# NeRdTheNed/deft4j

Hardware: NVIDIA B200
Metric: input MB/s optimised (-m NONE) (higher is better)
Workload: dtype u8

## Files before the change

__graft_entry__.py:

```python
import os
import subprocess
import sys

ROOT = os.path.dirname(os.path.abspath(__file__))
CSRC = os.path.join(ROOT, "deft4j_b200", "csrc")
NVCC = os.environ.get("NVCC", "/usr/local/cuda/bin/nvcc")


def _newer(target, sources):
    if not os.path.exists(target):
        return True
    t = os.path.getmtime(target)
    return any(os.path.exists(s) and os.path.getmtime(s) > t for s in sources)


def build():
    srcs = [os.path.join(CSRC, f) for f in os.listdir(CSRC) if f.endswith((".cu", ".cuh", ".cpp", ".h"))]
    srcs.append(os.path.join(ROOT, "include", "deft4cu.h"))
    lib = os.path.join(ROOT, "deft4j_b200", "libdeft4cu.so")
    if _newer(lib, srcs):
        subprocess.check_call([NVCC, "-gencode", "arch=compute_100a,code=sm_100a", "-O3", "-lineinfo", "-std=c++17",
                               "--shared", "-Xcompiler", "-fPIC,-pthread", "-o", lib, os.path.join(CSRC, "deft4cu.cu"),
                               os.path.join(CSRC, "png_front.cpp"), os.path.join(CSRC, "zip_front.cpp"),
                               os.path.join(CSRC, "gz_front.cpp")])
    small = os.path.join(ROOT, "deft4j_b200", "libdeft4cu_smallpools.so")
    if _newer(small, srcs):
        subprocess.check_call([NVCC, "-gencode", "arch=compute_100a,code=sm_100a", "-O3", "-lineinfo", "-std=c++17",
                               "-DD4_SMALL_POOLS", "--shared", "-Xcompiler", "-fPIC,-pthread", "-o", small,
                               os.path.join(CSRC, "deft4cu.cu"), os.path.join(CSRC, "png_front.cpp"),
                               os.path.join(CSRC, "zip_front.cpp"), os.path.join(CSRC, "gz_front.cpp")])
    stress = os.path.join(ROOT, "deft4j_b200", "libdeft4cu_stress.so")
    if _newer(stress, srcs):
        subprocess.check_call([NVCC, "-gencode", "arch=compute_100a,code=sm_100a", "-O3", "-lineinfo", "-std=c++17",
                               "-DD4_HQS=40", "-DD4_HQL=8", "-DD4_LCN=2", "-DD4_DCN=2", "-DD4_MAXLIT=3",
                               "-DD4_FORCE_BIG_WEIGHTS", "--shared", "-Xcompiler", "-fPIC,-pthread", "-o", stress,
                               os.path.join(CSRC, "deft4cu.cu"), os.path.join(CSRC, "png_front.cpp"),
                               os.path.join(CSRC, "zip_front.cpp"), os.path.join(CSRC, "gz_front.cpp")])
    host = os.path.join(ROOT, "deft4j_b200", "libdeft4cu_hosttest.so")
    if _newer(host, srcs):
        subprocess.check_call([NVCC, "-O2", "-std=c++17", "--shared", "-Xcompiler", "-fPIC", "-Wno-deprecated-gpu-targets",
                               "-o", host, os.path.join(CSRC, "hosttest.cu")])
    subprocess.check_call(["make", "-C", os.path.join(ROOT, "oracle")], stdout=subprocess.DEVNULL)
    sys.path.insert(0, ROOT)
    sys.path.insert(0, os.path.join(ROOT, "tests"))
    import hosttest_lib
    hosttest_lib.front_oracle_lib()
    import deft4j_b200
    from deft4j_b200 import _native
    _native.load()


def smoke():
    sys.path.insert(0, ROOT)
    sys.path.insert(0, os.path.join(ROOT, "tests"))
    import zlib
    import workloads
    import oracle_lib
    from deft4j_b200 import optimise_batch, _native
    if not os.path.exists(_native.LIB_PATH):
        build()
    co = zlib.compressobj(6, zlib.DEFLATED, -15, 8)
    cf = zlib.compressobj(6, zlib.DEFLATED, -15, 8, zlib.Z_FIXED)
    text = workloads.c2_text(60000)
    streams = [co.compress(text) + co.flush(), cf.compress(text[:3000]) + cf.flush()]
    res = optimise_batch(streams, True)
    for raw, r in zip(streams, res):
        assert r["status"] == 0, r
        o = oracle_lib.OracleDeflateStream()
# ... 25 lines not shown
```

deft4j_b200/csrc/deft4cu.cu:

```cuda
#include <algorithm>
#include <cstdio>
#include <cstdlib>
#include <cstring>
#include <memory>
#include <chrono>
#include <mutex>
#include <string>
#include <thread>
#include <vector>

#include "../../include/deft4cu.h"

namespace d4 {
static thread_local std::string g_err;
static void set_error(const std::string& s) { g_err = s; }
}

#include "write.cuh"
#include "checksum.cuh"

namespace d4 {

static int g_device = -1;
static int g_sms = 148;
static bool g_sync_debug = getenv("D4_SYNC") != nullptr;
static uint64_t g_opt_launches = 0;
static std::mutex g_mu;

struct HostTimer {
    const char* what; std::chrono::steady_clock::time_point t0; bool on;
    explicit HostTimer(const char* w) : what(w), t0(std::chrono::steady_clock::now()) { static bool e = getenv("D4_HOST_TIMING") != nullptr; on = e; }
    ~HostTimer() {
        if (on && g_device >= 0) {
            cudaMemPool_t pool;
            uint64_t res = 0, used = 0;
            if (cudaDeviceGetDefaultMemPool(&pool, g_device) == cudaSuccess) {
                cudaMemPoolGetAttribute(pool, cudaMemPoolAttrReservedMemCurrent, &res);
                cudaMemPoolGetAttribute(pool, cudaMemPoolAttrUsedMemCurrent, &used);
            }
            fprintf(stderr, "[deft4cu] pool reserved %7.1f MiB used %7.1f MiB  ", res / 1048576.0, used / 1048576.0);
        }
        if (on) fprintf(stderr, "[deft4cu] %-14s %8.3f ms\n", what, std::chrono::duration<double, std::milli>(std::chrono::steady_clock::now() - t0).count());
// ... 489 lines not shown
        cudaEventElapsedTime(&t, ev[0], ev[1]); ms[0] = t;
        cudaEventElapsedTime(&t, ev[1], ev[2]); ms[1] = t;
        cudaEventElapsedTime(&t, ev[2], ev[3]); ms[2] = t;
        ms[7] = (float)parse_rewalks;
        for (auto& e : ev) cudaEventDestroy(e);
        parsed = true;
        return DEFT4CU_OK;
    }

    unsigned char* scratch_raw = nullptr;
    cudaError_t alloc_scratch(EngScratch& sc, unsigned& grid, uint32_t maxwords, uint64_t maxu) {
        const size_t stride = eng_scratch_layout(sc, maxwords, maxu);
        const size_t align = (size_t)2 << 20;
        size_t freeb = 0, totalb = 0;
        if (cudaMemGetInfo(&freeb, &totalb) == cudaSuccess) {
            cudaMemPool_t pool;
            uint64_t res = 0, used = 0;
            if (cudaDeviceGetDefaultMemPool(&pool, g_device) == cudaSuccess &&
                cudaMemPoolGetAttribute(pool, cudaMemPoolAttrReservedMemCurrent, &res) == cudaSuccess &&
                cudaMemPoolGetAttribute(pool, cudaMemPoolAttrUsedMemCurrent, &used) == cudaSuccess && res > used)
                freeb += (size_t)(res - used);
            const size_t margin = ((size_t)1 << 30) + totalb / 16;
            const size_t fit = freeb > margin + align ? (freeb - margin - align) / stride : 0;
            grid = (unsigned)std::max<size_t>(1, std::min<size_t>(grid, fit));
        }
        cudaError_t e = dalloc(&scratch_raw, stride * grid + align, cs);
        if (e != cudaSuccess) return e;
        sc.slab = (unsigned char*)(((uintptr_t)scratch_raw + align - 1) & ~(uintptr_t)(align - 1));
        if (getenv("D4_POISON")) cudaMemsetAsync(sc.slab, 0x7F, stride * grid, cs);
        return cudaSuccess;
    }
    void free_scratch(EngScratch&) { dfree(scratch_raw, cs); }

    int optimise(uint32_t flags, const std::vector<uint8_t>& selected) {
        HostTimer ht("optimise");
        cudaEvent_t ev[3];
        for (auto& e : ev) cudaEventCreate(&e);
        const int merge = (flags & DEFT4CU_MERGE_BLOCKS) ? 1 : 0;
        if (optimised && nblk_total) {
            BlkSummary* d_summ = nullptr;
            D4_CUDA_CHECK(dalloc(&d_summ, nblk_total, cs));
            LAUNCH(k_state_summary, (unsigned)((nblk_total + 255) / 256), 256, cs, d_bs, d_summ, nblk_total);
            D4_CUDA_CHECK(cudaMemcpyAsync(summ.data(), d_summ, sizeof(BlkSummary) * nblk_total, cudaMemcpyDeviceToHost, cs));
            D4_CUDA_CHECK(cudaStreamSynchronize(cs));
            dfree(d_summ, cs);
        }
        optimised = true;
        std::vector<uint32_t> jobs;
        uint32_t maxsym = 1, maxstream = 1;
        uint64_t maxout = 1, maxstream_out = 1;
        for (uint32_t i = 0; i < n; i++) {
            StreamState& s = sstate[i];
            s.selected = selected[i] && s.status == ST_OK;
            s.saved_bits = 0;
            if (!s.selected) continue;
            uint64_t ssum = 0;
            uint32_t n_alive = 0;
            for (uint32_t k = 0; k < s.n_blocks; k++) n_alive += summ[s.blk_base + k].alive;
            s.cut = s.n_blocks;
            for (uint32_t k = 0; k < s.n_blocks; k++) {
                const BlkSummary& b = summ[s.blk_base + k];
                if (b.alive && b.out_len == 0 && n_alive != 1) { s.cut = k; break; }
            }
            for (uint32_t k = 0; k < s.n_blocks; k++) {
                const BlkSummary& b = summ[s.blk_base + k];
                ssum += b.n_sym;
// ... 2 lines not shown
                    maxsym = std::max(maxsym, b.n_sym);
                    maxout = std::max<uint64_t>(maxout, b.out_len);
                }
            }
            maxstream = (uint32_t)std::max<uint64_t>(maxstream, ssum);
            maxstream_out = std::max<uint64_t>(maxstream_out, infos[i].out_len);
        }
        const bool tracing = g_trace_dev != nullptr;
        if (!tracing) std::stable_sort(jobs.begin(), jobs.end(), [&](uint32_t a, uint32_t b) { return summ[a].n_sym > summ[b].n_sym; });
        D4_CUDA_CHECK(cudaMemcpyAsync(d_sstate, sstate.data(), sizeof(StreamState) * n, cudaMemcpyHostToDevice, cs));
        cudaEventRecord(ev[0], cs);
        if (!jobs.empty()) {
            uint32_t* d_jobs = nullptr;
            unsigned* d_counter = nullptr;
            D4_CUDA_CHECK(dalloc(&d_jobs, jobs.size(), cs));
            D4_CUDA_CHECK(dalloc(&d_counter, 1, cs));
            D4_CUDA_CHECK(cudaMemsetAsync(d_counter, 0, 4, cs));
            D4_CUDA_CHECK(cudaMemcpyAsync(d_jobs, jobs.data(), 4 * jobs.size(), cudaMemcpyHostToDevice, cs));
            int perSM = 0;
            cudaFuncSetAttribute(k_opt_blocks, cudaFuncAttributePreferredSharedMemoryCarveout, cudaSharedmemCarveoutMaxShared);
            D4_CUDA_CHECK(cudaOccupancyMaxActiveBlocksPerMultiprocessor(&perSM, k_opt_blocks, ENG_NT, 0));
            if (perSM < 1) perSM = 1;
            if (const char* e = getenv("D4_CTAS_PER_SM")) perSM = std::max(1, std::min(perSM, atoi(e)));
            unsigned grid = (unsigned)std::min<uint64_t>(jobs.size(), (uint64_t)g_sms * perSM);
            if (tracing) grid = 1;
            EngScratch sc{};
            D4_CUDA_CHECK(alloc_scratch(sc, grid, (maxsym + 31) / 32 + 1, maxout));
            g_opt_launches++;
            LAUNCH(k_opt_blocks, grid, ENG_NT, cs, d_jobs, (uint32_t)jobs.size(), d_bs, d_logs, d_sym, d_symout, d_out, d_maskpool, sc, d_counter, d_gerr);
            free_scratch(sc);
            dfree(d_jobs, cs); dfree(d_counter, cs);
        }
        cudaEventRecord(ev[1], cs);
        {
            EngScratch sc{};
            int perSM = 0;
            cudaFuncSetAttribute(k_finish, cudaFuncAttributePreferredSharedMemoryCarveout, cudaSharedmemCarveoutMaxShared);
            D4_CUDA_CHECK(cudaOccupancyMaxActiveBlocksPerMultiprocessor(&perSM, k_finish, ENG_NT, 0));
            if (perSM < 1) perSM = 1;
            unsigned grid = (unsigned)std::min<uint64_t>(n, (uint64_t)g_sms * perSM);
            unsigned* d_counter = nullptr;
            D4_CUDA_CHECK(dalloc(&d_counter, 1, cs));
            D4_CUDA_CHECK(cudaMemsetAsync(d_counter, 0, 4, cs));
            if (merge) D4_CUDA_CHECK(alloc_scratch(sc, grid, (maxstream + 31) / 32 + 2, maxstream_out));
            if (n) LAUNCH(k_finish, grid, ENG_NT, cs, d_sstate, n, d_bs, d_logs, d_sym, d_symout, d_out, d_maskpool, sc, merge, d_counter, d_gerr);
            if (merge) free_scratch(sc);
            dfree(d_counter, cs);
        }
        cudaEventRecord(ev[2], cs);
        int gerrv[8] = {0};
        D4_CUDA_CHECK(cudaMemcpyAsync(sstate.data(), d_sstate, sizeof(StreamState) * n, cudaMemcpyDeviceToHost, cs));
        D4_CUDA_CHECK(cudaMemcpyAsync(gerrv, d_gerr, sizeof(gerrv), cudaMemcpyDeviceToHost, cs));
        D4_CUDA_CHECK(cudaStreamSynchronize(cs));
        float t;
        cudaEventElapsedTime(&t, ev[0], ev[1]); ms[3] = t;
        cudaEventElapsedTime(&t, ev[1], ev[2]); ms[4] = t;
        for (auto& e : ev) cudaEventDestroy(e);
        const int gerr = gerrv[0];
        if (gerr == 13 || gerr == 14) {
            char msg[256];
            snprintf(msg, sizeof msg, "engine self-check: block %d round %d winner idx %d selected size %d, materialised size %d (check %d: 1 "
                     "incumbent != previous winner, 2 payload, 3 size; previous %d; %zu jobs)",
                     gerrv[1], gerrv[2], gerrv[3], gerrv[4], gerrv[5], gerrv[6], gerrv[7], jobs.size());
            set_error(msg);
            return DEFT4CU_ERR_CUDA;
        }
        if (gerr) {
            set_error(gerr == ERR_ROUNDS ? "optimiser hit an internal limit: more than 64 optimiseBlock rounds on one block"
                      : gerr == ERR_POOL ? "optimiser: internal table pool overflow"
                      : gerr == ERR_INTERNAL ? "optimiser: enumerator/executor protocol error (internal)"
                                         : "optimiser: a Huffman tree could not be balanced (the reference throws here)");
            D4_CUDA_CHECK(cudaMemsetAsync(d_gerr, 0, sizeof(int), cs));
            for (uint32_t i = 0; i < n; i++) if (sstate[i].selected) sstate[i].status = ST_UNSUPPORTED;
            return DEFT4CU_ERR_UNSUPPORTED;
        }
        dfree(d_dst, cs);
        h_dst.clear();
        return DEFT4CU_OK;
    }

// ... 503 lines not shown
```

deft4j_b200/csrc/optimise.cuh:

```cuda
#pragma once
#include "engine.cuh"

namespace d4 {

constexpr int MAXR = 64;

struct BlkState {
    Cand cand;
    uint64_t sym_off;
    uint64_t out_off;
    uint64_t mask_off;
    uint64_t out_len;
    uint32_t n_sym;
    int32_t alive;
    int32_t bfinal;
    int32_t nrounds;
    uint64_t bit_pos;
    long long size_bits;
};
struct RoundRec { long long sizeI, sizeC1, restMin, best; };
struct RoundLog { RoundRec r[MAXR]; };

struct StreamState {
    uint64_t blk_base;
// ... 86 lines not shown
                e.pass_hist_full(SLOT_BEST);
                const long long truePay = e.hist_payload(S.hist, e.recs[1].tab);
                if (truePay != e.recs[1].payload) { bad = true; badWhat = 2; }
                if (cand_size(e.recs[1]) != S.en.bestSize) { bad = true; badWhat = 3; }
            }
            if (bad && tid == 0) {
                if (atomicMax(gerr, 13) < 13) {
                    gerr[1] = (int)jobs[job]; gerr[2] = r; gerr[3] = (int)S.en.bestIndex;
                    gerr[4] = (int)S.en.bestSize; gerr[5] = (int)cand_size(e.recs[1]); gerr[6] = badWhat; gerr[7] = (int)prevBest;
                }
            }
            __syncthreads();
            prevBest = S.en.bestSize;
            r++;
            if (!improved) break;
            if (r >= MAXR) { if (tid == 0) S.err = ERR_ROUNDS; break; }
            e.advance_to_best();
        }
        __syncthreads();
        if (r > 1 && !S.err) {
            const uint32_t* s = (const uint32_t*)&e.recs[0];
            uint32_t* d = (uint32_t*)&b.cand;
            for (int k = tid; k < (int)(sizeof(Cand) / 4); k += ENG_NT) d[k] = s[k];
            e.store_mask(SLOT_B, maskpool + b.mask_off);
        }
        if (tid == 0) b.nrounds = r;
        __syncthreads();
        if (S.err) { if (tid == 0) { atomicMax(gerr, S.err); S.err = 0; } }
        __syncthreads();
        P1(PR_BLOCK);
    }
}

__device__ void finish_stream(EngSmem& S, Eng& e, StreamState& st, BlkState* __restrict__ bs, const RoundLog* __restrict__ logs,
                              uint32_t* __restrict__ sym, const uint32_t* __restrict__ symout, const uint8_t* __restrict__ out,
                              uint32_t* __restrict__ maskpool, int merge, int* __restrict__ gerr) {
    __shared__ long long s_pos, s_saved;
    __shared__ int s_cur, s_next, s_do, s_first;
    if (!st.selected || st.status != ST_OK) return;
    const int tid = threadIdx.x;
    BlkState* B = bs + st.blk_base;
    const uint32_t nb = st.n_blocks;

    {
        constexpr int RT = 64, RR = 4;
        struct Tile { unsigned long long out_len[RT]; int type[RT]; RoundRec rr[RT][RR]; };
        static_assert(sizeof(Tile) <= sizeof(EngSmem), "replay tile must fit in the engine's shared storage");
        Tile& T = *reinterpret_cast<Tile*>(&S);
        __shared__ long long s_rpos, s_rsaved;
        __shared__ int s_stop;
        __shared__ uint32_t s_first_alive, s_n_alive;
        if (tid == 0) { s_rpos = 0; s_rsaved = 0; s_stop = 0; s_first_alive = nb; s_n_alive = 0; }
        __syncthreads();
        {
            uint32_t fa = nb, na = 0;
            for (uint32_t k = tid; k < nb; k += ENG_NT) if (B[k].alive) { if (fa == nb) fa = k; na++; }
            if (na) { atomicMin(&s_first_alive, fa); atomicAdd(&s_n_alive, na); }
        }
        __syncthreads();
        const uint32_t first_alive = s_first_alive, n_alive = s_n_alive;
        for (uint32_t t0 = 0; t0 < nb && !s_stop; t0 += RT) {
            const uint32_t cnt = nb - t0 < RT ? nb - t0 : RT;
            for (uint32_t k = tid; k < cnt; k += ENG_NT) {
                T.out_len[k] = B[t0 + k].out_len;
                T.type[k] = B[t0 + k].alive ? (int)B[t0 + k].cand.tab.type : -1;
            }
            for (uint32_t q = tid; q < cnt * RR; q += ENG_NT) T.rr[q / RR][q % RR] = logs[st.blk_base + t0 + q / RR].r[q % RR];
            __syncthreads();
            if (tid == 0) {
                long long pos = s_rpos, saved = s_rsaved;
                for (uint32_t kk = 0; kk < cnt; kk++) {
                    const uint32_t k = t0 + kk;
                    const unsigned long long out_len = T.out_len[kk];
                    if (T.type[kk] < 0) continue;
                    if (out_len > 0 || (k == first_alive && n_alive == 1)) {
                        if (T.type[kk] == 0) {
                            pos += 3;
                            pos += stored_size(out_len, pos);
                        } else {
                            const RoundLog& lg = logs[st.blk_base + k];
                            int r = 0;
                            while (true) {
                                pos += 3;
                                const RoundRec rr = r < RR ? T.rr[kk][r] : lg.r[r];
                                const long long I = rr.sizeI, C1 = rr.sizeC1, R = rr.restMin, W = rr.best;
                                const long long m1 = I < C1 ? I : C1;
                                bool storedWins = false;
                                long long Ssz = 0;
                                if (out_len <= 65535) {
                                    Ssz = stored_size(out_len, pos);
                                    storedWins = Ssz < m1 && Ssz <= R;
                                }
                                if (storedWins) {
                                    saved += I - Ssz;
                                    B[k].cand.tab.type = 0;
                                    pos += stored_size(out_len, pos);
                                    pos += 3;
                                    pos += stored_size(out_len, pos);
                                    break;
                                }
                                if (W < I) { saved += I - W; pos += W; r++; continue; }
                                pos += I;
                                break;
                            }
                        }
                    } else {
                        saved += blk_size(B[k], pos + 3) + 3;
                        B[k].alive = 0;
                        if (B[k].cand.tab.type != 0 && B[k].n_sym) sym[B[k].sym_off + B[k].n_sym - 1] = SYM_NOP;
                        s_stop = 1;
                        break;
                    }
                }
                s_rpos = pos; s_rsaved = saved;
            }
            __syncthreads();
        }
        if (tid == 0) { s_saved = s_rsaved; S.err = 0; }
    }
    __syncthreads();

    if (merge) {
        if (tid == 0) {
            s_pos = 0; s_first = 1;
            int c = 0;
            while (c < (int)nb && !B[c].alive) c++;
            s_cur = c;
        }
        __syncthreads();
        while (true) {
            const int cur = s_cur;
            if (cur >= (int)nb) break;
            if (tid == 0) {
                int n = cur + 1;
                while (n < (int)nb && !B[n].alive) n++;
                s_next = n < (int)nb ? n : -1;
                s_do = 0;
                BlkState& c = B[cur];
                if (s_first && s_next < 0) {
                    s_pos += blk_size(c, s_pos + 3) + 3;
                    s_do = 3;
                } else if (c.out_len > 0) {
                    s_pos += 3;
                    if (s_next >= 0) {
                        BlkState& nx = B[s_next];
                        if (c.cand.tab.type == 0) {
                            if (c.out_len + nx.out_len <= 65535) {
                                long long curSize = blk_size(c, s_pos);
                                long long nextSize = blk_size(nx, s_pos + curSize + 3);
                                long long mergedSize = stored_size(c.out_len + nx.out_len, s_pos);
                                long long cs = curSize + 3 + nextSize - mergedSize;
                                if (cs > 0) {
                                    s_saved += cs;
                                    c.out_len += nx.out_len;
                                    c.n_sym = 0;
// ... 46 lines not shown
                }
                __syncthreads();
                if (s_do == 5) {
                    if (!S.en.bestStored) {
                        const uint32_t* s = (const uint32_t*)&e.recs[1];
                        uint32_t* d = (uint32_t*)&c.cand;
                        for (int k = tid; k < (int)(sizeof(Cand) / 4); k += ENG_NT) d[k] = s[k];
                        e.store_mask(SLOT_BEST, maskpool + c.mask_off);
                    }
                    __syncthreads();
                    if (tid == 0) {
                        if (S.en.bestStored) c.cand.tab.type = 0;
                        c.n_sym = span;
                        c.out_len += nx.out_len;
                        nx.alive = 0;
                    }
                } else {
                    if (tid == 0) sym[c.sym_off + nA - 1] = 256;
                }
                __syncthreads();
                if (tid == 0) s_pos += blk_size(c, s_pos);
                action = (s_do == 5) ? 2 : 3;
                __syncthreads();
            }
            if (action == 4) break;
            if (tid == 0) {
                if (action == 3) {
                    s_cur = s_next < 0 ? (int)nb : s_next;
                    s_first = 0;
                }
            }
            __syncthreads();
        }
        if (S.err && tid == 0) { atomicMax(gerr, S.err); S.err = 0; }
    }
    __syncthreads();

    {
        constexpr int LT = 128;
        struct LTile { unsigned long long out_len[LT], bit_pos[LT]; long long csize[LT], size_bits[LT]; int type[LT], alive[LT]; };
        static_assert(sizeof(LTile) <= sizeof(EngSmem), "layout tile must fit in the engine's shared storage");
        __syncthreads();
        LTile& T = *reinterpret_cast<LTile*>(&S);
        __shared__ long long s_size;
        __shared__ int s_last;
        if (tid == 0) { s_size = 0; s_last = -1; }
        __syncthreads();
        for (uint32_t t0 = 0; t0 < nb; t0 += LT) {
            const uint32_t cnt = nb - t0 < LT ? nb - t0 : LT;
            for (uint32_t k = tid; k < cnt; k += ENG_NT) {
                const BlkState& b = B[t0 + k];
                T.out_len[k] = b.out_len; T.type[k] = b.cand.tab.type; T.alive[k] = b.alive; T.csize[k] = cand_size(b.cand);
            }
            __syncthreads();
            if (tid == 0) {
                long long size = s_size;
                int last = s_last;
                for (uint32_t k = 0; k < cnt; k++) {
                    if (!T.alive[k]) continue;
                    T.bit_pos[k] = (unsigned long long)size;
                    size += 3;
                    T.size_bits[k] = T.type[k] == 0 ? stored_size(T.out_len[k], size) : T.csize[k];
                    size += T.size_bits[k];
                    last = (int)(t0 + k);
                }
                s_size = size; s_last = last;
            }
            __syncthreads();
            for (uint32_t k = tid; k < cnt; k += ENG_NT) {
                if (!T.alive[k]) continue;
                BlkState& b = B[t0 + k];
                b.bit_pos = T.bit_pos[k]; b.size_bits = T.size_bits[k]; b.bfinal = 0;
            }
            __syncthreads();
        }
        if (tid == 0) {
            if (s_last >= 0) B[s_last].bfinal = 1;
            st.total_bits = (uint64_t)s_size;
            st.saved_bits = s_saved;
        }
        __syncthreads();
    }
}

__global__ void __launch_bounds__(ENG_NT, D4_ENG_MINB)
k_finish(StreamState* __restrict__ streams, uint32_t nstreams, BlkState* __restrict__ bs, const RoundLog* __restrict__ logs,
         uint32_t* __restrict__ sym, const uint32_t* __restrict__ symout, const uint8_t* __restrict__ out,
         uint32_t* __restrict__ maskpool, EngScratch sc, int merge, unsigned* __restrict__ counter, int* __restrict__ gerr) {
    EngSmem& S = g_es;
    __shared__ uint32_t s_job;
    Eng e;
    if (merge) eng_init(e, sc, blockIdx.x);
    while (true) {
        __syncthreads();
        if (threadIdx.x == 0) s_job = atomicAdd(counter, 1u);
        __syncthreads();
        const uint32_t job = s_job;
        if (job >= nstreams) break;
        finish_stream(S, e, streams[job], bs, logs, sym, symout, out, maskpool, merge, gerr);
    }
}

}
```

deft4j_b200/csrc/write.cuh:

```cuda
#pragma once
#include "optimise.cuh"

namespace d4 {

constexpr int WR_NT = 256;

__device__ __forceinline__ void put_bits(unsigned long long* outw, uint64_t bitpos, unsigned long long bits, int n) {
    if (n == 0) return;
    const uint64_t w = bitpos >> 6;
    const int sh = (int)(bitpos & 63);
    atomicOr(&outw[w], bits << sh);
    if (sh + n > 64) atomicOr(&outw[w + 1], bits >> (64 - sh));
}

__device__ __forceinline__ uint32_t rev_bits(uint32_t code, int len) { return len ? (__brev(code) >> (32 - len)) : 0; }

__device__ inline void build_codes(const uint8_t* lens, int n, uint16_t* codes) {
    int count[16];
    for (int l = 0; l < 16; l++) count[l] = 0;
    for (int i = 0; i < n; i++) count[lens[i] & 15]++;
    uint32_t next[16];
    uint32_t nc = 0;
    int lastShift = 0;
    for (int l = 1; l < 16; l++) {
        next[l] = 0;
        if (count[l] == 0) continue;
        nc <<= (l - lastShift);
        lastShift = l;
        next[l] = nc;
        nc += count[l];
    }
    for (int i = 0; i < n; i++) {
        int l = lens[i];
        codes[i] = l ? (uint16_t)rev_bits(next[l]++, l) : 0;
    }
}

struct WriteSmem {
    uint16_t codeL[MAX_LL], codeD[MAX_D], codeCL[MAX_CL];
    uint8_t L[MAX_LL], D[MAX_D];
    uint32_t warpsum[WR_NT / 32];
    uint64_t base;
};

__global__ void __launch_bounds__(WR_NT)
k_write(const StreamState* __restrict__ streams, const uint32_t* __restrict__ blk_stream, const BlkState* __restrict__ bs,
        const uint32_t* __restrict__ sym, const uint32_t* __restrict__ symout, const uint8_t* __restrict__ out,
        const uint32_t* __restrict__ maskpool, const uint64_t* __restrict__ dst_off, unsigned long long* __restrict__ dstw,
        int* __restrict__ gerr) {
    const BlkState& b = bs[blockIdx.x];
    const uint32_t sid = blk_stream[blockIdx.x];
    if (!b.alive || streams[sid].status != ST_OK) return;
    const int tid = threadIdx.x;
    unsigned long long* dw = dstw + (dst_off[sid] >> 3);
    const uint64_t pos0 = b.bit_pos;
    const int type = b.cand.tab.type;

    if (type == 0) {
        const uint64_t dataByte = ((pos0 + 3 + 7) >> 3) + 4;
        const uint8_t* src = out + b.out_off;
        if (tid == 0) {
            put_bits(dw, pos0, (unsigned long long)(b.bfinal ? 1 : 0), 3);
            uint32_t len = (uint32_t)b.out_len & 0xffff;
            uint32_t hdr = len | ((~len & 0xffff) << 16);
            put_bits(dw, (dataByte - 4) * 8, hdr, 32);
        }
        const uint64_t n = b.out_len;
        for (uint64_t k = (uint64_t)tid * 8; k < n; k += (uint64_t)WR_NT * 8) {
            unsigned long long v = 0;
            int cnt = (int)((n - k) < 8 ? (n - k) : 8);
            for (int j = 0; j < cnt; j++) v |= (unsigned long long)src[k + j] << (8 * j);
            put_bits(dw, (dataByte + k) * 8, v, cnt * 8);
        }
        return;
    }

    __shared__ WriteSmem W;
    for (int k = tid; k < MAX_LL; k += WR_NT) W.L[k] = b.cand.tab.L[k];
    if (tid < MAX_D) W.D[tid] = b.cand.tab.D[tid];
    __syncthreads();
    if (tid == 0) {
        if (type == 1) { W.L[286] = 8; W.L[287] = 8; }
        build_codes(W.L, type == 1 ? 288 : b.cand.tab.nL, W.codeL);
    }
    if (tid == 32) build_codes(W.D, b.cand.tab.nD, W.codeD);
    if (tid == 64 && type == 2) build_codes(b.cand.hdr.CL, 19, W.codeCL);
    __syncthreads();

    if (tid == 0) {
        uint64_t p = pos0;
        put_bits(dw, p, (unsigned long long)((type << 1) | (b.bfinal ? 1 : 0)), 3);
        p += 3;
        if (type == 2) {
            const Hdr& h = b.cand.hdr;
            put_bits(dw, p, (unsigned long long)((b.cand.tab.nL - 257) & 31), 5); p += 5;
            put_bits(dw, p, (unsigned long long)((b.cand.tab.nD - 1) & 31), 5); p += 5;
            put_bits(dw, p, (unsigned long long)((h.ncl - 4) & 15), 4); p += 4;
            for (int i = 0; i < h.ncl; i++) { put_bits(dw, p, h.CL[c_codelen_order[i]], 3); p += 3; }
            for (int i = 0; i < h.np; i++) {
                uint16_t pr = h.pairs[i];
                int s = pair_sym(pr), run = pair_run(pr);
                put_bits(dw, p, W.codeCL[s], h.CL[s]); p += h.CL[s];
                if (run > 0) {
                    int off = s == 18 ? 11 : 3, sz = pair_extra_bits(s);
                    put_bits(dw, p, (unsigned long long)(run - off), sz); p += sz;
                }
            }
            if ((long long)(p - pos0 - 3) != (long long)h.bits) {
                if (atomicMax(gerr, 2) == 0) { gerr[1] = (int)blockIdx.x; gerr[2] = (int)(p - pos0 - 3); gerr[3] = h.bits; gerr[4] = 1; }
            }
        }
        W.base = p;
    }
    __syncthreads();

    const uint32_t* S = sym + b.sym_off;
    const uint32_t* SO = symout + b.sym_off;
    const uint32_t* M = maskpool + b.mask_off;
    const int lane = tid & 31, wid = tid >> 5;
    for (uint32_t base = 0; base < b.n_sym; base += WR_NT) {
        const uint32_t i = base + tid;
        uint32_t s = 0;
        int nbits = 0;
        bool replaced = false;
        if (i < b.n_sym) {
            s = S[i];
            if (!sym_is_match(s)) {
                nbits = (s <= 256) ? W.L[s] : 0;
            } else {
                replaced = (M[i >> 5] >> (i & 31)) & 1;
                if (!replaced) {
                    int ls = sym_lensym(s), ds = dist_sym(sym_dist(s));
                    nbits = W.L[ls] + len_ebits_of(ls) + W.D[ds] + dist_ebits_of(ds);
                } else {
                    const uint8_t* p = out + SO[i];
                    int len = sym_len(s);
                    for (int k = 0; k < len; k++) nbits += W.L[p[k]];
                }
            }
        }
        uint32_t incl = (uint32_t)nbits;
#pragma unroll
        for (int d = 1; d < 32; d <<= 1) {
            uint32_t a = __shfl_up_sync(0xffffffffu, incl, d);
            if (lane >= d) incl += a;
        }
        if (lane == 31) W.warpsum[wid] = incl;
        __syncthreads();
        uint32_t wbase = 0, total = 0;
        for (int k = 0; k < WR_NT / 32; k++) { uint32_t x = W.warpsum[k]; if (k < wid) wbase += x; total += x; }
        uint64_t p = W.base + wbase + incl - (uint32_t)nbits;
        if (i < b.n_sym && nbits) {
            if (!sym_is_match(s)) {
                put_bits(dw, p, W.codeL[s], nbits);
            } else if (!replaced) {
                int ls = sym_lensym(s), dist = sym_dist(s), ds = dist_sym(dist), len = sym_len(s);
                unsigned long long bits = W.codeL[ls];
                int nb = W.L[ls];
                bits |= (unsigned long long)(len - c_len_base[ls - 257]) << nb;
                nb += len_ebits_of(ls);
                bits |= (unsigned long long)W.codeD[ds] << nb;
                nb += W.D[ds];
                bits |= (unsigned long long)(dist - c_dist_base[ds]) << nb;
                nb += dist_ebits_of(ds);
                put_bits(dw, p, bits, nb);
            } else {
                const uint8_t* q = out + SO[i];
                int len = sym_len(s);
                unsigned long long acc = 0;
                int na = 0;
                for (int k = 0; k < len; k++) {
                    int v = q[k], l = W.L[v];
                    if (na + l > 64) { put_bits(dw, p, acc, na); p += na; acc = 0; na = 0; }
                    acc |= (unsigned long long)W.codeL[v] << na;
                    na += l;
                }
                put_bits(dw, p, acc, na);
            }
        }
        __syncthreads();
        if (tid == 0) W.base += total;
        __syncthreads();
    }
    if (tid == 0) {
        if ((long long)(W.base - pos0 - 3) != b.size_bits) {
            if (atomicMax(gerr, 2) == 0) { gerr[1] = (int)blockIdx.x; gerr[2] = (int)(W.base - pos0 - 3); gerr[3] = (int)b.size_bits; gerr[4] = 2; }
        }
    }
}

}
```

Measured before the change: 1338.

## Parallelise replay and layout via residue-map scans; stage bit writes in shared memory

The serial per-stream replay and layout that ran on one thread inside k_finish is replaced by per-block kernels. These compute bit-position-mod-8 transition maps, compose them with a CUB inclusive scan, and use an exclusive sum for block bit offsets. Separately, k_write now stages output bits in a shared-memory buffer using 32-bit shared atomics and flushes whole words with plain stores, falling back to global atomics when a chunk does not fit. The aim is to remove serial single-thread work and heavy global atomicOr traffic, at the cost of several extra launches, temporary allocations and more shared memory per write block.

```diff
diff --git a/__graft_entry__.py b/__graft_entry__.py
--- a/__graft_entry__.py
+++ b/__graft_entry__.py
@@ -33,7 +33,7 @@
     if _newer(stress, srcs):
         subprocess.check_call([NVCC, "-gencode", "arch=compute_100a,code=sm_100a", "-O3", "-lineinfo", "-std=c++17",
                                "-DD4_HQS=40", "-DD4_HQL=8", "-DD4_LCN=2", "-DD4_DCN=2", "-DD4_MAXLIT=3",
-                               "-DD4_FORCE_BIG_WEIGHTS", "--shared", "-Xcompiler", "-fPIC,-pthread", "-o", stress,
+                               "-DD4_FORCE_BIG_WEIGHTS", "-DD4_WR_BUF=8", "--shared", "-Xcompiler", "-fPIC,-pthread", "-o", stress,
                                os.path.join(CSRC, "deft4cu.cu"), os.path.join(CSRC, "png_front.cpp"),
                                os.path.join(CSRC, "zip_front.cpp"), os.path.join(CSRC, "gz_front.cpp")])
     host = os.path.join(ROOT, "deft4j_b200", "libdeft4cu_hosttest.so")
diff --git a/deft4j_b200/csrc/deft4cu.cu b/deft4j_b200/csrc/deft4cu.cu
--- a/deft4j_b200/csrc/deft4cu.cu
+++ b/deft4j_b200/csrc/deft4cu.cu
@@ -8,6 +8,8 @@
 #include <string>
 #include <thread>
 #include <vector>
+
+#include <cub/device/device_scan.cuh>
 
 #include "../../include/deft4cu.h"
 
@@ -563,6 +565,53 @@
     }
     void free_scratch(EngScratch&) { dfree(scratch_raw, cs); }
 
+    int scan_residues(uint32_t* d_map, uint32_t* d_scan) {
+        size_t tb = 0;
+        D4_CUDA_CHECK(cub::DeviceScan::InclusiveScan(nullptr, tb, d_map, d_scan, RmapThen{}, nblk_total, cs));
+        unsigned char* d_tmp = nullptr;
+        D4_CUDA_CHECK(dalloc(&d_tmp, tb, cs));
+        D4_CUDA_CHECK(cub::DeviceScan::InclusiveScan(d_tmp, tb, d_map, d_scan, RmapThen{}, nblk_total, cs));
+        launches++;
+        dfree(d_tmp, cs);
+        return DEFT4CU_OK;
+    }
+    int replay() {
+        const unsigned g = (unsigned)((nblk_total + 255) / 256);
+        ReplayRec* d_rec = nullptr;
+        uint32_t *d_map = nullptr, *d_scan = nullptr;
+        D4_CUDA_CHECK(dalloc(&d_rec, nblk_total, cs));
+        D4_CUDA_CHECK(dalloc(&d_map, nblk_total, cs));
+        D4_CUDA_CHECK(dalloc(&d_scan, nblk_total, cs));
+        LAUNCH(k_replay_map, g, 256, cs, d_sstate, d_blk_stream, d_bs, d_logs, d_rec, d_map, nblk_total);
+        if (int rc = scan_residues(d_map, d_scan)) return rc;
+        LAUNCH(k_replay_apply, g, 256, cs, d_sstate, d_blk_stream, d_bs, d_rec, d_scan, d_sym, nblk_total);
+        dfree(d_rec, cs); dfree(d_map, cs); dfree(d_scan, cs);
+        return DEFT4CU_OK;
+    }
+    int layout() {
+        const unsigned g = (unsigned)((nblk_total + 256) / 256);
+        uint32_t *d_map = nullptr, *d_scan = nullptr;
+        unsigned long long *d_len = nullptr, *d_pos = nullptr;
+        D4_CUDA_CHECK(dalloc(&d_map, nblk_total, cs));
+        D4_CUDA_CHECK(dalloc(&d_scan, nblk_total, cs));
+        D4_CUDA_CHECK(dalloc(&d_len, nblk_total + 1, cs));
+        D4_CUDA_CHECK(dalloc(&d_pos, nblk_total + 1, cs));
+        LAUNCH(k_layout_map, g, 256, cs, d_sstate, d_blk_stream, d_bs, d_map, nblk_total);
+        if (int rc = scan_residues(d_map, d_scan)) return rc;
+        LAUNCH(k_layout_size, g, 256, cs, d_sstate, d_blk_stream, d_bs, d_scan, d_len, nblk_total);
+        size_t tb = 0;
+        D4_CUDA_CHECK(cub::DeviceScan::ExclusiveSum(nullptr, tb, d_len, d_pos, nblk_total + 1, cs));
+        unsigned char* d_tmp = nullptr;
+        D4_CUDA_CHECK(dalloc(&d_tmp, tb, cs));
+        D4_CUDA_CHECK(cub::DeviceScan::ExclusiveSum(d_tmp, tb, d_len, d_pos, nblk_total + 1, cs));
+        launches++;
+        dfree(d_tmp, cs);
+        LAUNCH(k_layout_apply, g, 256, cs, d_sstate, d_blk_stream, d_bs, d_pos, nblk_total);
+        LAUNCH(k_layout_streams, (n + 255) / 256, 256, cs, d_sstate, d_pos, n);
+        dfree(d_map, cs); dfree(d_scan, cs); dfree(d_len, cs); dfree(d_pos, cs);
+        return DEFT4CU_OK;
+    }
+
     int optimise(uint32_t flags, const std::vector<uint8_t>& selected) {
         HostTimer ht("optimise");
         cudaEvent_t ev[3];
@@ -631,7 +680,11 @@
             dfree(d_jobs, cs); dfree(d_counter, cs);
         }
         cudaEventRecord(ev[1], cs);
-        {
+        if (nblk_total) {
+            const int rc = replay();
+            if (rc != DEFT4CU_OK) return rc;
+        }
+        if (merge && n) {
             EngScratch sc{};
             int perSM = 0;
             cudaFuncSetAttribute(k_finish, cudaFuncAttributePreferredSharedMemoryCarveout, cudaSharedmemCarveoutMaxShared);
@@ -641,10 +694,14 @@
             unsigned* d_counter = nullptr;
             D4_CUDA_CHECK(dalloc(&d_counter, 1, cs));
             D4_CUDA_CHECK(cudaMemsetAsync(d_counter, 0, 4, cs));
-            if (merge) D4_CUDA_CHECK(alloc_scratch(sc, grid, (maxstream + 31) / 32 + 2, maxstream_out));
-            if (n) LAUNCH(k_finish, grid, ENG_NT, cs, d_sstate, n, d_bs, d_logs, d_sym, d_symout, d_out, d_maskpool, sc, merge, d_counter, d_gerr);
-            if (merge) free_scratch(sc);
+            D4_CUDA_CHECK(alloc_scratch(sc, grid, (maxstream + 31) / 32 + 2, maxstream_out));
+            LAUNCH(k_finish, grid, ENG_NT, cs, d_sstate, n, d_bs, d_sym, d_symout, d_out, d_maskpool, sc, d_counter, d_gerr);
+            free_scratch(sc);
             dfree(d_counter, cs);
+        }
+        if (nblk_total) {
+            const int rc = layout();
+            if (rc != DEFT4CU_OK) return rc;
         }
         cudaEventRecord(ev[2], cs);
         int gerrv[8] = {0};
diff --git a/deft4j_b200/csrc/optimise.cuh b/deft4j_b200/csrc/optimise.cuh
--- a/deft4j_b200/csrc/optimise.cuh
+++ b/deft4j_b200/csrc/optimise.cuh
@@ -142,95 +142,193 @@
     }
 }
 
-__device__ void finish_stream(EngSmem& S, Eng& e, StreamState& st, BlkState* __restrict__ bs, const RoundLog* __restrict__ logs,
-                              uint32_t* __restrict__ sym, const uint32_t* __restrict__ symout, const uint8_t* __restrict__ out,
-                              uint32_t* __restrict__ maskpool, int merge, int* __restrict__ gerr) {
+constexpr uint32_t RMAP_ID = 0xFAC688u;
+constexpr uint32_t RMAP_CONST1 = 0x249249u;
+__host__ __device__ __forceinline__ uint32_t rmap_get(uint32_t m, uint32_t r) { return (m >> (3 * r)) & 7u; }
+struct RmapThen {
+    __host__ __device__ __forceinline__ uint32_t operator()(uint32_t a, uint32_t b) const {
+        uint32_t c = 0;
+#pragma unroll
+        for (uint32_t r = 0; r < 8; r++) c |= rmap_get(b, rmap_get(a, r)) << (3 * r);
+        return c;
+    }
+};
+
+constexpr uint32_t RP_STORED = 0xFFu;
+constexpr uint32_t RP_LIVE = 1u << 8;
+constexpr uint32_t RP_STOP = 1u << 9;
+struct ReplayRec { long long saved[8]; uint32_t flags; };
+
+__device__ __forceinline__ const StreamState* blk_home(const StreamState* st, const uint32_t* blk_stream, uint64_t i, uint32_t& k) {
+    const StreamState* s = st + blk_stream[i];
+    k = (uint32_t)(i - s->blk_base);
+    return s->selected && s->status == ST_OK ? s : nullptr;
+}
+__device__ __forceinline__ uint32_t rmap_head(uint32_t m, uint32_t k) { return k == 0 ? rmap_get(m, 0) * RMAP_CONST1 : m; }
+__device__ __forceinline__ uint32_t rmap_in(const uint32_t* scan, uint64_t i, uint32_t k) { return k == 0 ? 0 : rmap_get(scan[i - 1], 0); }
+
+__global__ void k_replay_map(const StreamState* __restrict__ st, const uint32_t* __restrict__ blk_stream,
+                             const BlkState* __restrict__ bs, const RoundLog* __restrict__ logs,
+                             ReplayRec* __restrict__ rec, uint32_t* __restrict__ rmap, uint64_t nblk) {
+    const uint64_t i = (uint64_t)blockIdx.x * blockDim.x + threadIdx.x;
+    if (i >= nblk) return;
+    uint32_t k;
+    const StreamState* s = blk_home(st, blk_stream, i, k);
+    const BlkState& b = bs[i];
+    uint32_t m = RMAP_ID, flags = 0;
+    if (s && k <= s->cut && b.alive) {
+        ReplayRec& R = rec[i];
+        if (k == s->cut) {
+            flags = RP_STOP;
+            for (int r = 0; r < 8; r++) R.saved[r] = blk_size(b, r + 3) + 3;
+        } else {
+            flags = RP_LIVE;
+            m = 0;
+            const uint64_t out_len = b.out_len;
+            for (int r0 = 0; r0 < 8; r0++) {
+                long long pos = r0, saved = 0;
+                if (b.cand.tab.type == 0) {
+                    pos += 3;
+                    pos += stored_size(out_len, pos);
+                } else {
+                    const RoundLog& lg = logs[i];
+                    int r = 0;
+                    while (true) {
+                        pos += 3;
+                        const RoundRec rr = lg.r[r];
+                        const long long I = rr.sizeI, C1 = rr.sizeC1, R = rr.restMin, W = rr.best;
+                        const long long m1 = I < C1 ? I : C1;
+                        bool storedWins = false;
+                        long long Ssz = 0;
+                        if (out_len <= 65535) {
+                            Ssz = stored_size(out_len, pos);
+                            storedWins = Ssz < m1 && Ssz <= R;
+                        }
+                        if (storedWins) {
+                            saved += I - Ssz;
+                            flags |= 1u << r0;
+                            pos += stored_size(out_len, pos);
+                            pos += 3;
+                            pos += stored_size(out_len, pos);
+                            break;
+                        }
+                        if (W < I) { saved += I - W; pos += W; r++; continue; }
+                        pos += I;
+                        break;
+                    }
+                }
+                m |= (uint32_t)(pos & 7) << (3 * r0);
+                R.saved[r0] = saved;
+            }
+        }
+    }
+    rmap[i] = rmap_head(m, k);
+    rec[i].flags = flags;
+}
+
+__device__ __forceinline__ long long warp_run_sum(long long v, uint32_t key, bool& leader) {
+    const unsigned peers = __match_any_sync(0xffffffffu, key);
+    const int lane = threadIdx.x & 31;
+#pragma unroll
+    for (int d = 1; d < 32; d <<= 1) {
+        const long long o = __shfl_down_sync(0xffffffffu, v, d);
+        if (lane + d < 32 && ((peers >> (lane + d)) & 1)) v += o;
+    }
+    leader = lane == __ffs(peers) - 1;
+    return v;
+}
+
+__global__ void k_replay_apply(StreamState* __restrict__ st, const uint32_t* __restrict__ blk_stream, BlkState* __restrict__ bs,
+                               const ReplayRec* __restrict__ rec, const uint32_t* __restrict__ scan, uint32_t* __restrict__ sym,
+                               uint64_t nblk) {
+    const uint64_t i = (uint64_t)blockIdx.x * blockDim.x + threadIdx.x;
+    long long saved = 0;
+    uint32_t sid = 0xFFFFFFFFu;
+    if (i < nblk) {
+        sid = blk_stream[i];
+        const uint32_t flags = rec[i].flags;
+        if (flags) {
+            const uint32_t k = (uint32_t)(i - st[sid].blk_base);
+            const uint32_t r = rmap_in(scan, i, k);
+            saved = rec[i].saved[r];
+            BlkState& b = bs[i];
+            if (flags & RP_STOP) {
+                b.alive = 0;
+                if (b.cand.tab.type != 0 && b.n_sym) sym[b.sym_off + b.n_sym - 1] = SYM_NOP;
+            } else if ((flags >> r) & 1) {
+                b.cand.tab.type = 0;
+            }
+        }
+    }
+    bool leader;
+    saved = warp_run_sum(saved, sid, leader);
+    if (leader && saved != 0) atomicAdd((unsigned long long*)&st[sid].saved_bits, (unsigned long long)saved);
+}
+
+__global__ void k_layout_map(const StreamState* __restrict__ st, const uint32_t* __restrict__ blk_stream,
+                             const BlkState* __restrict__ bs, uint32_t* __restrict__ rmap, uint64_t nblk) {
+    const uint64_t i = (uint64_t)blockIdx.x * blockDim.x + threadIdx.x;
+    if (i >= nblk) return;
+    uint32_t k;
+    const StreamState* s = blk_home(st, blk_stream, i, k);
+    const BlkState& b = bs[i];
+    uint32_t m = RMAP_ID;
+    if (s && b.alive) {
+        m = 0;
+        for (int r = 0; r < 8; r++) m |= (uint32_t)((r + 3 + blk_size(b, r + 3)) & 7) << (3 * r);
+    }
+    rmap[i] = rmap_head(m, k);
+}
+
+__global__ void k_layout_size(const StreamState* __restrict__ st, const uint32_t* __restrict__ blk_stream,
+                              BlkState* __restrict__ bs, const uint32_t* __restrict__ scan, unsigned long long* __restrict__ len,
+                              uint64_t nblk) {
+    const uint64_t i = (uint64_t)blockIdx.x * blockDim.x + threadIdx.x;
+    if (i > nblk) return;
+    unsigned long long l = 0;
+    if (i < nblk) {
+        uint32_t k;
+        const StreamState* s = blk_home(st, blk_stream, i, k);
+        BlkState& b = bs[i];
+        if (s && b.alive) {
+            b.size_bits = blk_size(b, rmap_in(scan, i, k) + 3);
+            l = 3 + (unsigned long long)b.size_bits;
+        }
+    }
+    len[i] = l;
+}
+
+__global__ void k_layout_apply(const StreamState* __restrict__ st, const uint32_t* __restrict__ blk_stream,
+                               BlkState* __restrict__ bs, const unsigned long long* __restrict__ pos, uint64_t nblk) {
+    const uint64_t i = (uint64_t)blockIdx.x * blockDim.x + threadIdx.x;
+    if (i >= nblk) return;
+    uint32_t k;
+    const StreamState* s = blk_home(st, blk_stream, i, k);
+    BlkState& b = bs[i];
+    if (!s || !b.alive) return;
+    b.bit_pos = pos[i] - pos[s->blk_base];
+    b.bfinal = pos[i + 1] == pos[s->blk_base + s->n_blocks] ? 1 : 0;
+}
+__global__ void k_layout_streams(StreamState* __restrict__ st, const unsigned long long* __restrict__ pos, uint32_t n) {
+    const uint32_t j = blockIdx.x * blockDim.x + threadIdx.x;
+    if (j >= n) return;
+    StreamState& s = st[j];
+    if (s.selected && s.status == ST_OK) s.total_bits = pos[s.blk_base + s.n_blocks] - pos[s.blk_base];
+}
+
+__device__ void merge_stream(EngSmem& S, Eng& e, StreamState& st, BlkState* __restrict__ bs,
+                             uint32_t* __restrict__ sym, const uint32_t* __restrict__ symout, const uint8_t* __restrict__ out,
+                             uint32_t* __restrict__ maskpool, int* __restrict__ gerr) {
     __shared__ long long s_pos, s_saved;
     __shared__ int s_cur, s_next, s_do, s_first;
     if (!st.selected || st.status != ST_OK) return;
     const int tid = threadIdx.x;
     BlkState* B = bs + st.blk_base;
     const uint32_t nb = st.n_blocks;
+    if (tid == 0) s_saved = st.saved_bits;
+    __syncthreads();
 
     {
-        constexpr int RT = 64, RR = 4;
-        struct Tile { unsigned long long out_len[RT]; int type[RT]; RoundRec rr[RT][RR]; };
-        static_assert(sizeof(Tile) <= sizeof(EngSmem), "replay tile must fit in the engine's shared storage");
-        Tile& T = *reinterpret_cast<Tile*>(&S);
-        __shared__ long long s_rpos, s_rsaved;
-        __shared__ int s_stop;
-        __shared__ uint32_t s_first_alive, s_n_alive;
-        if (tid == 0) { s_rpos = 0; s_rsaved = 0; s_stop = 0; s_first_alive = nb; s_n_alive = 0; }
-        __syncthreads();
-        {
-            uint32_t fa = nb, na = 0;
-            for (uint32_t k = tid; k < nb; k += ENG_NT) if (B[k].alive) { if (fa == nb) fa = k; na++; }
-            if (na) { atomicMin(&s_first_alive, fa); atomicAdd(&s_n_alive, na); }
-        }
-        __syncthreads();
-        const uint32_t first_alive = s_first_alive, n_alive = s_n_alive;
-        for (uint32_t t0 = 0; t0 < nb && !s_stop; t0 += RT) {
-            const uint32_t cnt = nb - t0 < RT ? nb - t0 : RT;
-            for (uint32_t k = tid; k < cnt; k += ENG_NT) {
-                T.out_len[k] = B[t0 + k].out_len;
-                T.type[k] = B[t0 + k].alive ? (int)B[t0 + k].cand.tab.type : -1;
-            }
-            for (uint32_t q = tid; q < cnt * RR; q += ENG_NT) T.rr[q / RR][q % RR] = logs[st.blk_base + t0 + q / RR].r[q % RR];
-            __syncthreads();
-            if (tid == 0) {
-                long long pos = s_rpos, saved = s_rsaved;
-                for (uint32_t kk = 0; kk < cnt; kk++) {
-                    const uint32_t k = t0 + kk;
-                    const unsigned long long out_len = T.out_len[kk];
-                    if (T.type[kk] < 0) continue;
-                    if (out_len > 0 || (k == first_alive && n_alive == 1)) {
-                        if (T.type[kk] == 0) {
-                            pos += 3;
-                            pos += stored_size(out_len, pos);
-                        } else {
-                            const RoundLog& lg = logs[st.blk_base + k];
-                            int r = 0;
-                            while (true) {
-                                pos += 3;
-                                const RoundRec rr = r < RR ? T.rr[kk][r] : lg.r[r];
-                                const long long I = rr.sizeI, C1 = rr.sizeC1, R = rr.restMin, W = rr.best;
-                                const long long m1 = I < C1 ? I : C1;
-                                bool storedWins = false;
-                                long long Ssz = 0;
-                                if (out_len <= 65535) {
-                                    Ssz = stored_size(out_len, pos);
-                                    storedWins = Ssz < m1 && Ssz <= R;
-                                }
-                                if (storedWins) {
-                                    saved += I - Ssz;
-                                    B[k].cand.tab.type = 0;
-                                    pos += stored_size(out_len, pos);
-                                    pos += 3;
-                                    pos += stored_size(out_len, pos);
-                                    break;
-                                }
-                                if (W < I) { saved += I - W; pos += W; r++; continue; }
-                                pos += I;
-                                break;
-                            }
-                        }
-                    } else {
-                        saved += blk_size(B[k], pos + 3) + 3;
-                        B[k].alive = 0;
-                        if (B[k].cand.tab.type != 0 && B[k].n_sym) sym[B[k].sym_off + B[k].n_sym - 1] = SYM_NOP;
-                        s_stop = 1;
-                        break;
-                    }
-                }
-                s_rpos = pos; s_rsaved = saved;
-            }
-            __syncthreads();
-        }
-        if (tid == 0) { s_saved = s_rsaved; S.err = 0; }
-    }
-    __syncthreads();
-
-    if (merge) {
         if (tid == 0) {
             s_pos = 0; s_first = 1;
             int c = 0;
@@ -343,73 +441,30 @@
             }
             __syncthreads();
         }
-        if (S.err && tid == 0) { atomicMax(gerr, S.err); S.err = 0; }
+        if (tid == 0) {
+            if (S.err) { atomicMax(gerr, S.err); S.err = 0; }
+            st.saved_bits = s_saved;
+        }
     }
     __syncthreads();
-
-    {
-        constexpr int LT = 128;
-        struct LTile { unsigned long long out_len[LT], bit_pos[LT]; long long csize[LT], size_bits[LT]; int type[LT], alive[LT]; };
-        static_assert(sizeof(LTile) <= sizeof(EngSmem), "layout tile must fit in the engine's shared storage");
-        __syncthreads();
-        LTile& T = *reinterpret_cast<LTile*>(&S);
-        __shared__ long long s_size;
-        __shared__ int s_last;
-        if (tid == 0) { s_size = 0; s_last = -1; }
-        __syncthreads();
-        for (uint32_t t0 = 0; t0 < nb; t0 += LT) {
-            const uint32_t cnt = nb - t0 < LT ? nb - t0 : LT;
-            for (uint32_t k = tid; k < cnt; k += ENG_NT) {
-                const BlkState& b = B[t0 + k];
-                T.out_len[k] = b.out_len; T.type[k] = b.cand.tab.type; T.alive[k] = b.alive; T.csize[k] = cand_size(b.cand);
-            }
-            __syncthreads();
-            if (tid == 0) {
-                long long size = s_size;
-                int last = s_last;
-                for (uint32_t k = 0; k < cnt; k++) {
-                    if (!T.alive[k]) continue;
-                    T.bit_pos[k] = (unsigned long long)size;
-                    size += 3;
-                    T.size_bits[k] = T.type[k] == 0 ? stored_size(T.out_len[k], size) : T.csize[k];
-                    size += T.size_bits[k];
-                    last = (int)(t0 + k);
-                }
-                s_size = size; s_last = last;
-            }
-            __syncthreads();
-            for (uint32_t k = tid; k < cnt; k += ENG_NT) {
-                if (!T.alive[k]) continue;
-                BlkState& b = B[t0 + k];
-                b.bit_pos = T.bit_pos[k]; b.size_bits = T.size_bits[k]; b.bfinal = 0;
-            }
-            __syncthreads();
-        }
-        if (tid == 0) {
-            if (s_last >= 0) B[s_last].bfinal = 1;
-            st.total_bits = (uint64_t)s_size;
-            st.saved_bits = s_saved;
-        }
-        __syncthreads();
-    }
 }
 
 __global__ void __launch_bounds__(ENG_NT, D4_ENG_MINB)
-k_finish(StreamState* __restrict__ streams, uint32_t nstreams, BlkState* __restrict__ bs, const RoundLog* __restrict__ logs,
+k_finish(StreamState* __restrict__ streams, uint32_t nstreams, BlkState* __restrict__ bs,
          uint32_t* __restrict__ sym, const uint32_t* __restrict__ symout, const uint8_t* __restrict__ out,
-         uint32_t* __restrict__ maskpool, EngScratch sc, int merge, unsigned* __restrict__ counter, int* __restrict__ gerr) {
+         uint32_t* __restrict__ maskpool, EngScratch sc, unsigned* __restrict__ counter, int* __restrict__ gerr) {
     EngSmem& S = g_es;
     __shared__ uint32_t s_job;
     Eng e;
-    if (merge) eng_init(e, sc, blockIdx.x);
+    eng_init(e, sc, blockIdx.x);
     while (true) {
         __syncthreads();
         if (threadIdx.x == 0) s_job = atomicAdd(counter, 1u);
         __syncthreads();
         const uint32_t job = s_job;
         if (job >= nstreams) break;
-        finish_stream(S, e, streams[job], bs, logs, sym, symout, out, maskpool, merge, gerr);
-    }
-}
-
-}
+        merge_stream(S, e, streams[job], bs, sym, symout, out, maskpool, gerr);
+    }
+}
+
+}
diff --git a/deft4j_b200/csrc/write.cuh b/deft4j_b200/csrc/write.cuh
--- a/deft4j_b200/csrc/write.cuh
+++ b/deft4j_b200/csrc/write.cuh
@@ -4,6 +4,10 @@
 namespace d4 {
 
 constexpr int WR_NT = 256;
+#ifndef D4_WR_BUF
+#define D4_WR_BUF 1024
+#endif
+constexpr int WR_BUF = D4_WR_BUF;
 
 __device__ __forceinline__ void put_bits(unsigned long long* outw, uint64_t bitpos, unsigned long long bits, int n) {
     if (n == 0) return;
@@ -11,6 +15,21 @@
     const int sh = (int)(bitpos & 63);
     atomicOr(&outw[w], bits << sh);
     if (sh + n > 64) atomicOr(&outw[w + 1], bits >> (64 - sh));
+}
+
+__device__ __forceinline__ void put_bits_s(unsigned long long* buf, uint64_t w0, uint64_t bitpos, unsigned long long bits, int n) {
+    if (n == 0) return;
+    uint32_t* b = reinterpret_cast<uint32_t*>(buf);
+    const uint32_t w = (uint32_t)((bitpos >> 5) - 2 * w0);
+    const int sh = (int)(bitpos & 31);
+    atomicOr(&b[w], (uint32_t)(bits << sh));
+    if (sh + n > 32) atomicOr(&b[w + 1], (uint32_t)(bits >> (32 - sh)));
+    if (sh + n > 64) atomicOr(&b[w + 2], (uint32_t)(bits >> (64 - sh)));
+}
+__device__ __forceinline__ void put_bits_w(bool fits, unsigned long long* buf, uint64_t w0, unsigned long long* dw, uint64_t bitpos,
+                                           unsigned long long bits, int n) {
+    if (fits) put_bits_s(buf, w0, bitpos, bits, n);
+    else put_bits(dw, bitpos, bits, n);
 }
 
 __device__ __forceinline__ uint32_t rev_bits(uint32_t code, int len) { return len ? (__brev(code) >> (32 - len)) : 0; }
@@ -41,7 +60,29 @@
     uint8_t L[MAX_LL], D[MAX_D];
     uint32_t warpsum[WR_NT / 32];
     uint64_t base;
+    unsigned long long buf[WR_BUF];
 };
+
+__device__ __forceinline__ bool wr_fits(WriteSmem& W, unsigned long long* dw, uint64_t w0, uint64_t end) {
+    if ((end >> 6) - w0 < (uint64_t)WR_BUF) return true;
+    if (threadIdx.x == 0 && W.buf[0]) { atomicOr(&dw[w0], W.buf[0]); W.buf[0] = 0; }
+    return false;
+}
+__device__ __forceinline__ uint64_t wr_flush(WriteSmem& W, unsigned long long* dw, uint64_t w0, uint64_t end, bool fits) {
+    const uint64_t w1 = end >> 6;
+    __syncthreads();
+    if (!fits) return w1;
+    const uint32_t nfull = (uint32_t)(w1 - w0);
+    for (uint32_t j = threadIdx.x; j < nfull; j += WR_NT) {
+        const unsigned long long v = W.buf[j];
+        if (j) dw[w0 + j] = v;
+        else if (v) atomicOr(&dw[w0], v);
+    }
+    const unsigned long long carry = W.buf[nfull];
+    __syncthreads();
+    for (uint32_t j = threadIdx.x; j <= nfull; j += WR_NT) W.buf[j] = j ? 0ull : carry;
+    return w1;
+}
 
 __global__ void __launch_bounds__(WR_NT)
 k_write(const StreamState* __restrict__ streams, const uint32_t* __restrict__ blk_stream, const BlkState* __restrict__ bs,
@@ -78,6 +119,7 @@
     __shared__ WriteSmem W;
     for (int k = tid; k < MAX_LL; k += WR_NT) W.L[k] = b.cand.tab.L[k];
     if (tid < MAX_D) W.D[tid] = b.cand.tab.D[tid];
+    for (int k = tid; k < WR_BUF; k += WR_NT) W.buf[k] = 0;
     __syncthreads();
     if (tid == 0) {
         if (type == 1) { W.L[286] = 8; W.L[287] = 8; }
@@ -87,23 +129,26 @@
     if (tid == 64 && type == 2) build_codes(b.cand.hdr.CL, 19, W.codeCL);
     __syncthreads();
 
+    uint64_t w0 = pos0 >> 6;
+    bool fits = wr_fits(W, dw, w0, pos0 + 74 + 14ull * (type == 2 ? b.cand.hdr.np : 0));
     if (tid == 0) {
+        auto put = [&](uint64_t q, unsigned long long bits, int n) { put_bits_w(fits, W.buf, w0, dw, q, bits, n); };
         uint64_t p = pos0;
-        put_bits(dw, p, (unsigned long long)((type << 1) | (b.bfinal ? 1 : 0)), 3);
+        put(p, (unsigned long long)((type << 1) | (b.bfinal ? 1 : 0)), 3);
         p += 3;
         if (type == 2) {
             const Hdr& h = b.cand.hdr;
-            put_bits(dw, p, (unsigned long long)((b.cand.tab.nL - 257) & 31), 5); p += 5;
-            put_bits(dw, p, (unsigned long long)((b.cand.tab.nD - 1) & 31), 5); p += 5;
-            put_bits(dw, p, (unsigned long long)((h.ncl - 4) & 15), 4); p += 4;
-            for (int i = 0; i < h.ncl; i++) { put_bits(dw, p, h.CL[c_codelen_order[i]], 3); p += 3; }
+            put(p, (unsigned long long)((b.cand.tab.nL - 257) & 31), 5); p += 5;
+            put(p, (unsigned long long)((b.cand.tab.nD - 1) & 31), 5); p += 5;
+            put(p, (unsigned long long)((h.ncl - 4) & 15), 4); p += 4;
+            for (int i = 0; i < h.ncl; i++) { put(p, h.CL[c_codelen_order[i]], 3); p += 3; }
             for (int i = 0; i < h.np; i++) {
                 uint16_t pr = h.pairs[i];
                 int s = pair_sym(pr), run = pair_run(pr);
-                put_bits(dw, p, W.codeCL[s], h.CL[s]); p += h.CL[s];
+                put(p, W.codeCL[s], h.CL[s]); p += h.CL[s];
                 if (run > 0) {
                     int off = s == 18 ? 11 : 3, sz = pair_extra_bits(s);
-                    put_bits(dw, p, (unsigned long long)(run - off), sz); p += sz;
+                    put(p, (unsigned long long)(run - off), sz); p += sz;
                 }
             }
             if ((long long)(p - pos0 - 3) != (long long)h.bits) {
@@ -112,6 +157,8 @@
         }
         W.base = p;
     }
+    __syncthreads();
+    w0 = wr_flush(W, dw, w0, W.base, fits);
     __syncthreads();
 
     const uint32_t* S = sym + b.sym_off;
@@ -149,10 +196,14 @@
         __syncthreads();
         uint32_t wbase = 0, total = 0;
         for (int k = 0; k < WR_NT / 32; k++) { uint32_t x = W.warpsum[k]; if (k < wid) wbase += x; total += x; }
-        uint64_t p = W.base + wbase + incl - (uint32_t)nbits;
+        const uint64_t tbase = W.base;
+        fits = wr_fits(W, dw, w0, tbase + total);
+        __syncthreads();
+        auto put = [&](uint64_t q, unsigned long long bits, int n) { put_bits_w(fits, W.buf, w0, dw, q, bits, n); };
+        uint64_t p = tbase + wbase + incl - (uint32_t)nbits;
         if (i < b.n_sym && nbits) {
             if (!sym_is_match(s)) {
-                put_bits(dw, p, W.codeL[s], nbits);
+                put(p, W.codeL[s], nbits);
             } else if (!replaced) {
                 int ls = sym_lensym(s), dist = sym_dist(s), ds = dist_sym(dist), len = sym_len(s);
                 unsigned long long bits = W.codeL[ls];
@@ -163,7 +214,7 @@
                 nb += W.D[ds];
                 bits |= (unsigned long long)(dist - c_dist_base[ds]) << nb;
                 nb += dist_ebits_of(ds);
-                put_bits(dw, p, bits, nb);
+                put(p, bits, nb);
             } else {
                 const uint8_t* q = out + SO[i];
                 int len = sym_len(s);
@@ -171,17 +222,18 @@
                 int na = 0;
                 for (int k = 0; k < len; k++) {
                     int v = q[k], l = W.L[v];
-                    if (na + l > 64) { put_bits(dw, p, acc, na); p += na; acc = 0; na = 0; }
+                    if (na + l > 64) { put(p, acc, na); p += na; acc = 0; na = 0; }
                     acc |= (unsigned long long)W.codeL[v] << na;
                     na += l;
                 }
-                put_bits(dw, p, acc, na);
-            }
-        }
+                put(p, acc, na);
+            }
+        }
+        w0 = wr_flush(W, dw, w0, tbase + total, fits);
+        if (tid == 0) W.base = tbase + total;
         __syncthreads();
-        if (tid == 0) W.base += total;
-        __syncthreads();
-    }
+    }
+    if (tid == 0 && W.buf[0]) atomicOr(&dw[w0], W.buf[0]);
     if (tid == 0) {
         if ((long long)(W.base - pos0 - 3) != b.size_bits) {
             if (atomicMax(gerr, 2) == 0) { gerr[1] = (int)blockIdx.x; gerr[2] = (int)(W.base - pos0 - 3); gerr[3] = (int)b.size_bits; gerr[4] = 2; }
```

Measured after the change: 1361 (median of 6 runs). +1.7%, better.
